# GeekAlexis/FastMOT

Measured on AMD Instinct MI355X. Metric: end-to-end tracker FPS @1080p/50 dets, higher is better.
Workload: dtype f16

## Files before the change

fastmot_amd/csrc/resblock.hip:

```cpp
#include "net.h"
#include <cstdlib>

namespace {

typedef float f32x16 __attribute__((ext_vector_type(16)));

template <int C, int M, int TH, int NW, int CS, int KS>
__global__ __launch_bounds__(NW * 64) void resblock_kernel(
    const f16* __restrict__ x, int x_cs, int x_coff, f16* __restrict__ out, int out_cs, int out_coff,
    const f16* __restrict__ w1, const float* __restrict__ b1, const f16* __restrict__ w2,
    const float* __restrict__ b2, int H, int W, int tiles_x, int act1, int act2) {
    constexpr int TW = 8, HW = TW + 2, NPOS = (TH + 2) * HW, SX = C + 8, S = M + 8, NT = NW * 64;
    constexpr int NMT = M / 32, NPH = (NPOS + 31) / 32, NPAIR = NMT * NPH / NW;
    constexpr int NCT = C / 32 / CS, NPT = TH * TW / 32;
    static_assert(NMT * NPH % NW == 0 && NCT * NPT * KS == NW, "tile / wave split");
    extern __shared__ __attribute__((aligned(16))) f16 lds[];
    f16* xt = lds;
    f16* mid = lds + NPOS * SX;
    const int tid = threadIdx.x, lane = tid & 63, wave = __builtin_amdgcn_readfirstlane(tid >> 6);
    const int frow = lane & 31, fk = (lane >> 5) * 8;
    const int tile = blockIdx.x / CS, cs = blockIdx.x % CS;
    const int ty0 = (tile / tiles_x) * TH, tx0 = (tile % tiles_x) * TW;
    const long n = blockIdx.y;
    const f16* img = x + n * (long)H * W * x_cs + x_coff;

    {
        constexpr int VPP = C / 8, NV = NPOS * VPP, NIT = (NV + NT - 1) / NT;
        f16x8 v[NIT];
#pragma unroll
        for (int i = 0; i < NIT; ++i) {
            const int e = tid + i * NT, pos = e / VPP, c8 = (e % VPP) * 8;
            const int py = ty0 - 1 + pos / HW, px = tx0 - 1 + pos % HW;
            const bool ok = e < NV && py >= 0 && py < H && px >= 0 && px < W;
            const f16x8 ld = *reinterpret_cast<const f16x8*>(
                img + ((long)min(max(py, 0), H - 1) * W + min(max(px, 0), W - 1)) * x_cs + c8);
#pragma unroll
            for (int j = 0; j < 8; ++j) v[i][j] = ok ? ld[j] : (f16)0.f;
        }
#pragma unroll
        for (int i = 0; i < NIT; ++i) {
            const int e = tid + i * NT;
            if (e < NV) *reinterpret_cast<f16x8*>(&xt[(e / VPP) * SX + (e % VPP) * 8]) = v[i];
        }
    }

    {
        constexpr int ST = C / 16, CH1 = ST < 8 ? ST : 8, KC = ST / CH1, NI = NPAIR * KC, PD = NI < 3 ? NI : 3;
        f16x8 fa[PD][CH1];
        float4 bias1[NPAIR][4];
#pragma unroll
        for (int p = 0; p < NPAIR; ++p)
#pragma unroll
            for (int g = 0; g < 4; ++g)
                bias1[p][g] = *reinterpret_cast<const float4*>((const float*)__builtin_assume_aligned(b1, 16) +
                                                               ((wave + p * NW) % NMT) * 32 + g * 8 + (lane >> 5) * 4);
        auto load_a = [&](int item, int slot) {
            const int mt = (wave + (item / KC) * NW) % NMT;
            const f16* wr = w1 + (((long)mt * ST + (item % KC) * CH1) * 64 + lane) * 8;
#pragma unroll
            for (int u = 0; u < CH1; ++u) fa[slot][u] = *reinterpret_cast<const f16x8*>(wr + u * 512);
        };
#pragma unroll
        for (int i = 0; i < PD; ++i) load_a(i, i);
        __syncthreads();
        f32x16 acc;
#pragma unroll
        for (int item = 0; item < NI; ++item) {
            const int p = item / KC, kc = (item % KC) * CH1 * 16;
            const int pos = ((wave + p * NW) / NMT) * 32 + frow;
            const f16* bsrc = xt + min(pos, NPOS - 1) * SX + fk + kc;
            f16x8 fb[CH1];
#pragma unroll
            for (int u = 0; u < CH1; ++u) fb[u] = *reinterpret_cast<const f16x8*>(bsrc + u * 16);
            if (item % KC == 0) {
#pragma unroll
                for (int r = 0; r < 16; ++r) acc[r] = 0.f;
            }
#pragma unroll
            for (int u = 0; u < CH1; ++u) acc = __builtin_amdgcn_mfma_f32_32x32x16_f16(fa[item % PD][u], fb[u], acc, 0, 0, 0);
            if (item + PD < NI) load_a(item + PD, item % PD);
            if (item % KC == KC - 1 && pos < NPOS) {
                const int py = ty0 - 1 + pos / HW, px = tx0 - 1 + pos % HW;
                const bool inside = py >= 0 && py < H && px >= 0 && px < W;
                const int mt = (wave + p * NW) % NMT;
#pragma unroll
                for (int g = 0; g < 4; ++g) {
                    const float4 bv = bias1[p][g];
                    union { f16 h[4]; uint2 u; } pk;
                    float a4[4] = {acc[g * 4 + 0] + bv.x, acc[g * 4 + 1] + bv.y, acc[g * 4 + 2] + bv.z,
                                   acc[g * 4 + 3] + bv.w};
                    apply_act_n<4>(a4, act1);
#pragma unroll
                    for (int e = 0; e < 4; ++e) pk.h[e] = (f16)(inside ? a4[e] : 0.f);
                    *reinterpret_cast<uint2*>(&mid[pos * S + mt * 32 + g * 8 + (lane >> 5) * 4]) = pk.u;
                }
            }
        }
    }

    const int ctl = wave % NCT, pt = (wave / NCT) % NPT, ks = wave / (NCT * NPT);
    const int ct = cs * NCT + ctl;
    const int pix = pt * 32 + frow;
    const int gy = ty0 + pix / TW, gx = tx0 + pix % TW;
    float4 bias2[4];
#pragma unroll
    for (int g = 0; g < 4; ++g)
        bias2[g] = *reinterpret_cast<const float4*>((const float*)__builtin_assume_aligned(b2, 16) + ct * 32 + g * 8 +
                                                    (lane >> 5) * 4);
    f32x16 acc;
    {
        constexpr int SPT = M / 16;
        constexpr int CH = (SPT % 8 == 0 && 9 * SPT % (8 * KS) == 0) ? 8 : (SPT % 4 == 0 && 9 * SPT % (4 * KS) == 0) ? 4 : 2;
        constexpr int NQ = 9 * SPT / CH / KS, PD = NQ < 24 / CH ? NQ : 24 / CH;
        static_assert(SPT % CH == 0 && 9 * SPT % (CH * KS) == 0, "chunking");
        const int q0 = ks * NQ;
        const f16* wr = w2 + (((long)ct * (9 * SPT) + q0 * CH) * 64 + lane) * 8;
        f16x8 fa[PD][CH], fb[2][CH];
        auto load_a = [&](int q, int slot) {
#pragma unroll
            for (int u = 0; u < CH; ++u) fa[slot][u] = *reinterpret_cast<const f16x8*>(wr + (q * CH + u) * 512);
        };
        const int pbase = ((pix / TW) * HW + pix % TW) * S + fk;
        auto load_b = [&](int q, int slot) {
            const int step0 = (q0 + q) * CH, tap = step0 / SPT;
            const f16* src = mid + pbase + ((tap / 3) * HW + tap % 3) * S + (step0 % SPT) * 16;
#pragma unroll
            for (int u = 0; u < CH; ++u) fb[slot][u] = *reinterpret_cast<const f16x8*>(src + u * 16);
        };
#pragma unroll
        for (int i = 0; i < PD; ++i) load_a(i, i);
#pragma unroll
        for (int r = 0; r < 16; ++r) acc[r] = 0.f;
        __syncthreads();
        load_b(0, 0);
#pragma unroll
        for (int q = 0; q < NQ; ++q) {
            if (q + 1 < NQ) load_b(q + 1, (q + 1) & 1);
            __builtin_amdgcn_sched_barrier(0);
#pragma unroll
            for (int u = 0; u < CH; ++u)
                acc = __builtin_amdgcn_mfma_f32_32x32x16_f16(fa[q % PD][u], fb[q & 1][u], acc, 0, 0, 0);
            if (q + PD < NQ) load_a(q + PD, q % PD);
            __builtin_amdgcn_sched_barrier(0);
        }
    }
    if constexpr (KS > 1) {
        float4* red = reinterpret_cast<float4*>(mid);
        __syncthreads();
        if (ks > 0) {
#pragma unroll
            for (int g = 0; g < 4; ++g)
                red[(((ks - 1) * NCT * NPT + ctl + NCT * pt) * 4 + g) * 64 + lane] =
                    make_float4(acc[g * 4], acc[g * 4 + 1], acc[g * 4 + 2], acc[g * 4 + 3]);
        }
        __syncthreads();
        if (ks > 0) return;
#pragma unroll
        for (int k = 1; k < KS; ++k)
#pragma unroll
            for (int g = 0; g < 4; ++g) {
                const float4 v = red[(((k - 1) * NCT * NPT + ctl + NCT * pt) * 4 + g) * 64 + lane];
                acc[g * 4] += v.x; acc[g * 4 + 1] += v.y; acc[g * 4 + 2] += v.z; acc[g * 4 + 3] += v.w;
            }
    }

    if (gy < H && gx < W) {
        const long gp = (n * H + gy) * (long)W + gx;
        const f16* rsrc = xt + ((pix / TW + 1) * HW + pix % TW + 1) * SX;
#pragma unroll
        for (int g = 0; g < 4; ++g) {
            const int co = ct * 32 + g * 8 + (lane >> 5) * 4;
            const f16x4 rv = *reinterpret_cast<const f16x4*>(rsrc + co);
            f16x4 o;
            float a4[4] = {acc[g * 4 + 0] + bias2[g].x, acc[g * 4 + 1] + bias2[g].y, acc[g * 4 + 2] + bias2[g].z,
                           acc[g * 4 + 3] + bias2[g].w};
            apply_act_n<4>(a4, act2);
#pragma unroll
            for (int e = 0; e < 4; ++e) o[e] = (f16)(a4[e] + (float)rv[e]);
            *reinterpret_cast<f16x4*>(out + gp * out_cs + out_coff + co) = o;
        }
    }
}

template <int C, int M, int TH, int NW, int KS>
constexpr size_t resblock_lds() {
    constexpr size_t npos = (TH + 2) * 10, midb = npos * (M + 8) * 2, redb = (size_t)(KS - 1) * (NW / KS) * 64 * 64;
    return npos * (C + 8) * 2 + (midb > redb ? midb : redb);
}

template <int C, int M, int TH, int NW, int CS, int KS>
int resblock_launch(const f16* x, int x_cs, int x_coff, f16* out, int out_cs, int out_coff, const f16* w1,
                    const float* b1, const f16* w2, const float* b2, int N, int H, int W, int act1, int act2,
                    hipStream_t s) {
    const int tiles_x = (W + 7) / 8, tiles_y = (H + TH - 1) / TH;
    constexpr size_t shmem = resblock_lds<C, M, TH, NW, KS>();
    static_assert(shmem <= 64 * 1024, "LDS tile");
    hipLaunchKernelGGL((resblock_kernel<C, M, TH, NW, CS, KS>), dim3(tiles_x * tiles_y * CS, N), dim3(NW * 64), shmem, s, x, x_cs,
                       x_coff, out, out_cs, out_coff, w1, b1, w2, b2, H, W, tiles_x, act1, act2);
    FM_HIP(hipGetLastError());
    return 0;
}

}

bool resblock_supported(int C, int M) {
    return (C == 64 || C == 128 || C == 256) && (M == C || M == C / 2);
}

int launch_resblock(const f16* x, int x_cs, int x_coff, f16* out, int out_cs, int out_coff, const f16* w1,
                    const float* b1, const f16* w2, const float* b2, int N, int H, int W, int C, int M, int act1,
                    int act2, hipStream_t s) {
    FM_CHECK_ARG(resblock_supported(C, M) && x_cs % 8 == 0 && x_coff % 8 == 0 && out_cs % 4 == 0 && out_coff % 4 == 0);
#define RB(C_, M_, TH_, NW_, CS_, KS_)                                                                         \
    if (C == C_ && M == M_)                                                                                    \
        return resblock_launch<C_, M_, TH_, NW_, CS_, KS_>(x, x_cs, x_coff, out, out_cs, out_coff, w1, b1, w2, \
                                                           b2, N, H, W, act1, act2, s)
    static const int variant = getenv("FASTMOT_RB_VARIANT") ? atoi(getenv("FASTMOT_RB_VARIANT")) : 1;
    if (variant == 1) { RB(64, 64, 8, 8, 1, 2); RB(128, 128, 4, 8, 1, 2); }
    if (variant == 2) { RB(128, 128, 8, 8, 1, 1); }
    RB(64, 32, 8, 4, 1, 1);
    RB(64, 64, 8, 4, 1, 1);
    RB(128, 64, 4, 4, 1, 1);
    RB(128, 128, 4, 4, 1, 1);
    RB(256, 128, 4, 8, 4, 4);
    RB(256, 256, 4, 8, 4, 4);
#undef RB
    return FM_ERR_ARG;
}

extern "C" int fm_resblock_supported(int c, int mid) { return resblock_supported(c, mid) ? 1 : 0; }
```

Measured before the change: 1027.

## Add persistent weight-resident resblock kernel with halo prefetch for C=64,M=32

Adds a persistent-style resblock kernel for C=64, M=32. Each block loops over a contiguous range of tiles, keeps both 1x1 and 3x3 weights in registers for the whole range, and prefetches the next tile's halo into registers while the 3x3 MFMA stage runs. The output is staged through LDS so global stores are 16-byte vectors. This is meant to cut repeated weight loads and hide global-load latency, at the cost of more registers and fewer blocks (about 512), which lowers occupancy and parallelism.

```diff
diff --git a/fastmot_amd/csrc/resblock.hip b/fastmot_amd/csrc/resblock.hip
--- a/fastmot_amd/csrc/resblock.hip
+++ b/fastmot_amd/csrc/resblock.hip
@@ -182,6 +182,193 @@
     }
 }
 
+#ifndef FM_RB_SLOTS
+#define FM_RB_SLOTS 512
+#endif
+#ifndef FM_RB_PREFETCH
+#define FM_RB_PREFETCH 1
+#endif
+
+template <int C, int M, int NW, int KS>
+__global__ __launch_bounds__(NW * 64) void resblock_lm_kernel(
+    const f16* __restrict__ x, int x_cs, int x_coff, f16* __restrict__ out, int out_cs, int out_coff,
+    const f16* __restrict__ w1, const float* __restrict__ b1, const f16* __restrict__ w2,
+    const float* __restrict__ b2, int H, int W, int tiles_x, int tiles_img, int tiles_total, int tpw, int act1,
+    int act2) {
+    constexpr int TH = 8, TW = 8, HW = TW + 2, NPOS = (TH + 2) * HW, SX = C + 8, S = M + 8, NT = NW * 64;
+    constexpr int NMT = M / 32, NPH = (NPOS + 31) / 32, NCT = C / 32, NPT = TH * TW / 32;
+    constexpr int ST = C / 16, SPT = M / 16, CH = 2, NQ = 9 * SPT / CH / KS;
+    static_assert(NMT * NPH == NW && NCT * NPT * KS == NW && 9 * SPT % (CH * KS) == 0 && ST == 4, "tile / wave split");
+    static_assert((SPT % 4 != 0 || 9 * SPT % (4 * KS) != 0) && NQ * CH <= 24, "chunking of resblock_kernel");
+    extern __shared__ __attribute__((aligned(16))) f16 lds[];
+    f16* xt = lds;
+    f16* mid = lds + NPOS * SX;
+    const int tid = threadIdx.x, lane = tid & 63, wave = __builtin_amdgcn_readfirstlane(tid >> 6);
+    const int frow = lane & 31, fk = (lane >> 5) * 8;
+    const int t0 = blockIdx.x * tpw, t1 = min(t0 + tpw, tiles_total);
+    if (t0 >= t1) return;
+
+    const int mt = wave % NMT, pos1 = (wave / NMT) * 32 + frow;
+    const int ct = wave % NCT, pt = (wave / NCT) % NPT, ks = wave / (NCT * NPT);
+    const int pix = pt * 32 + frow;
+    f16x8 fa1[ST], fa2[NQ][CH];
+    float4 bias1[4], bias2[4];
+#pragma unroll
+    for (int g = 0; g < 4; ++g) {
+        bias1[g] = *reinterpret_cast<const float4*>((const float*)__builtin_assume_aligned(b1, 16) + mt * 32 + g * 8 + (lane >> 5) * 4);
+        bias2[g] = *reinterpret_cast<const float4*>((const float*)__builtin_assume_aligned(b2, 16) + ct * 32 + g * 8 + (lane >> 5) * 4);
+    }
+#pragma unroll
+    for (int u = 0; u < ST; ++u) fa1[u] = *reinterpret_cast<const f16x8*>(w1 + (((long)mt * ST + u) * 64 + lane) * 8);
+#pragma unroll
+    for (int q = 0; q < NQ; ++q)
+#pragma unroll
+        for (int u = 0; u < CH; ++u)
+            fa2[q][u] = *reinterpret_cast<const f16x8*>(w2 + (((long)ct * (9 * SPT) + (ks * NQ + q) * CH + u) * 64 + lane) * 8);
+
+    constexpr int VPP = C / 8, NV = NPOS * VPP, NIT = (NV + NT - 1) / NT;
+    f16x8 hv[NIT];
+    unsigned hok = 0;
+    auto halo_load = [&](int t) {
+        const int n = t / tiles_img, r = t - n * tiles_img;
+        const int ty0 = (r / tiles_x) * TH, tx0 = (r % tiles_x) * TW;
+        const f16* img = x + (long)n * H * W * x_cs + x_coff;
+        hok = 0;
+#pragma unroll
+        for (int i = 0; i < NIT; ++i) {
+            const int e = tid + i * NT, pos = e / VPP, c8 = (e % VPP) * 8;
+            const int py = ty0 - 1 + pos / HW, px = tx0 - 1 + pos % HW;
+            hok |= (e < NV && py >= 0 && py < H && px >= 0 && px < W ? 1u : 0u) << i;
+            hv[i] = *reinterpret_cast<const f16x8*>(
+                img + ((long)min(max(py, 0), H - 1) * W + min(max(px, 0), W - 1)) * x_cs + c8);
+        }
+    };
+    auto halo_store = [&]() {
+#pragma unroll
+        for (int i = 0; i < NIT; ++i) {
+            const int e = tid + i * NT;
+            f16x8 v = hv[i];
+            if (!((hok >> i) & 1u)) {
+#pragma unroll
+                for (int j = 0; j < 8; ++j) v[j] = (f16)0.f;
+            }
+            if (e < NV) *reinterpret_cast<f16x8*>(&xt[(e / VPP) * SX + (e % VPP) * 8]) = v;
+        }
+    };
+    halo_load(t0);
+
+    for (int t = t0; t < t1; ++t) {
+        const int n = t / tiles_img, r = t - n * tiles_img;
+        const int ty0 = (r / tiles_x) * TH, tx0 = (r % tiles_x) * TW;
+        if (!FM_RB_PREFETCH && t > t0) halo_load(t);
+        halo_store();
+        __syncthreads();
+
+        {
+            const f16* bsrc = xt + min(pos1, NPOS - 1) * SX + fk;
+            f16x8 fb[ST];
+#pragma unroll
+            for (int u = 0; u < ST; ++u) fb[u] = *reinterpret_cast<const f16x8*>(bsrc + u * 16);
+            f32x16 acc;
+#pragma unroll
+            for (int r16 = 0; r16 < 16; ++r16) acc[r16] = 0.f;
+#pragma unroll
+            for (int u = 0; u < ST; ++u) acc = __builtin_amdgcn_mfma_f32_32x32x16_f16(fa1[u], fb[u], acc, 0, 0, 0);
+            if (pos1 < NPOS) {
+                const int py = ty0 - 1 + pos1 / HW, px = tx0 - 1 + pos1 % HW;
+                const bool inside = py >= 0 && py < H && px >= 0 && px < W;
+#pragma unroll
+                for (int g = 0; g < 4; ++g) {
+                    const float4 bv = bias1[g];
+                    union { f16 h[4]; uint2 u; } pk;
+                    float a4[4] = {acc[g * 4 + 0] + bv.x, acc[g * 4 + 1] + bv.y, acc[g * 4 + 2] + bv.z,
+                                   acc[g * 4 + 3] + bv.w};
+                    apply_act_n<4>(a4, act1);
+#pragma unroll
+                    for (int e = 0; e < 4; ++e) pk.h[e] = (f16)(inside ? a4[e] : 0.f);
+                    *reinterpret_cast<uint2*>(&mid[pos1 * S + mt * 32 + g * 8 + (lane >> 5) * 4]) = pk.u;
+                }
+            }
+        }
+        __syncthreads();
+        if (FM_RB_PREFETCH && t + 1 < t1) halo_load(t + 1);
+
+        f32x16 acc;
+        {
+            f16x8 fb[2][CH];
+            const int pbase = ((pix / TW) * HW + pix % TW) * S + fk;
+            auto load_b = [&](int q, int slot) {
+                const int step0 = (ks * NQ + q) * CH, tap = step0 / SPT;
+                const f16* src = mid + pbase + ((tap / 3) * HW + tap % 3) * S + (step0 % SPT) * 16;
+#pragma unroll
+                for (int u = 0; u < CH; ++u) fb[slot][u] = *reinterpret_cast<const f16x8*>(src + u * 16);
+            };
+#pragma unroll
+            for (int r16 = 0; r16 < 16; ++r16) acc[r16] = 0.f;
+            load_b(0, 0);
+#pragma unroll
+            for (int q = 0; q < NQ; ++q) {
+                if (q + 1 < NQ) load_b(q + 1, (q + 1) & 1);
+                __builtin_amdgcn_sched_barrier(0);
+#pragma unroll
+                for (int u = 0; u < CH; ++u)
+                    acc = __builtin_amdgcn_mfma_f32_32x32x16_f16(fa2[q][u], fb[q & 1][u], acc, 0, 0, 0);
+                __builtin_amdgcn_sched_barrier(0);
+            }
+        }
+        if constexpr (KS > 1) {
+            float4* red = reinterpret_cast<float4*>(mid);
+            __syncthreads();
+            if (ks > 0) {
+#pragma unroll
+                for (int g = 0; g < 4; ++g)
+                    red[(((ks - 1) * NCT * NPT + ct + NCT * pt) * 4 + g) * 64 + lane] =
+                        make_float4(acc[g * 4], acc[g * 4 + 1], acc[g * 4 + 2], acc[g * 4 + 3]);
+            }
+            __syncthreads();
+            if (ks == 0) {
+#pragma unroll
+                for (int k = 1; k < KS; ++k)
+#pragma unroll
+                    for (int g = 0; g < 4; ++g) {
+                        const float4 v = red[(((k - 1) * NCT * NPT + ct + NCT * pt) * 4 + g) * 64 + lane];
+                        acc[g * 4] += v.x; acc[g * 4 + 1] += v.y; acc[g * 4 + 2] += v.z; acc[g * 4 + 3] += v.w;
+                    }
+            }
+        }
+
+        if (ks == 0) {
+            f16* rsrc = xt + ((pix / TW + 1) * HW + pix % TW + 1) * SX;
+#pragma unroll
+            for (int g = 0; g < 4; ++g) {
+                const int co = ct * 32 + g * 8 + (lane >> 5) * 4;
+                const f16x4 rv = *reinterpret_cast<const f16x4*>(rsrc + co);
+                f16x4 o;
+                float a4[4] = {acc[g * 4 + 0] + bias2[g].x, acc[g * 4 + 1] + bias2[g].y, acc[g * 4 + 2] + bias2[g].z,
+                               acc[g * 4 + 3] + bias2[g].w};
+                apply_act_n<4>(a4, act2);
+#pragma unroll
+                for (int e = 0; e < 4; ++e) o[e] = (f16)(a4[e] + (float)rv[e]);
+                *reinterpret_cast<f16x4*>(rsrc + co) = o;
+            }
+        }
+        __syncthreads();
+        {
+            constexpr int NO = TH * TW * VPP;
+            static_assert(NO % NT == 0, "output pieces per thread");
+#pragma unroll
+            for (int i = 0; i < NO / NT; ++i) {
+                const int e = tid + i * NT, p = e / VPP, c8 = (e % VPP) * 8;
+                const int gy = ty0 + p / TW, gx = tx0 + p % TW;
+                if (gy < H && gx < W)
+                    *reinterpret_cast<f16x8*>(out + (((long)n * H + gy) * W + gx) * out_cs + out_coff + c8) =
+                        *reinterpret_cast<const f16x8*>(&xt[((p / TW + 1) * HW + p % TW + 1) * SX + c8]);
+            }
+        }
+        if (t + 1 < t1) __syncthreads();
+    }
+}
+
 template <int C, int M, int TH, int NW, int KS>
 constexpr size_t resblock_lds() {
     constexpr size_t npos = (TH + 2) * 10, midb = npos * (M + 8) * 2, redb = (size_t)(KS - 1) * (NW / KS) * 64 * 64;
@@ -201,6 +388,23 @@
     return 0;
 }
 
+template <int C, int M, int NW, int KS>
+int resblock_lm_launch(const f16* x, int x_cs, int x_coff, f16* out, int out_cs, int out_coff, const f16* w1,
+                       const float* b1, const f16* w2, const float* b2, int N, int H, int W, int act1, int act2,
+                       hipStream_t s) {
+    const int tiles_x = (W + 7) / 8, tiles_img = tiles_x * ((H + 7) / 8);
+    const long total = (long)tiles_img * N;
+    FM_CHECK_ARG(total < (1L << 30));
+    const int tpw = (int)((total + FM_RB_SLOTS - 1) / FM_RB_SLOTS);
+    constexpr size_t shmem = resblock_lds<C, M, 8, NW, KS>();
+    static_assert(shmem <= 64 * 1024, "LDS tile");
+    hipLaunchKernelGGL((resblock_lm_kernel<C, M, NW, KS>), dim3((unsigned)((total + tpw - 1) / tpw)), dim3(NW * 64), shmem, s, x,
+                       x_cs, x_coff, out, out_cs, out_coff, w1, b1, w2, b2, H, W, tiles_x, tiles_img, (int)total, tpw, act1,
+                       act2);
+    FM_HIP(hipGetLastError());
+    return 0;
+}
+
 }
 
 bool resblock_supported(int C, int M) {
@@ -216,6 +420,16 @@
         return resblock_launch<C_, M_, TH_, NW_, CS_, KS_>(x, x_cs, x_coff, out, out_cs, out_coff, w1, b1, w2, \
                                                            b2, N, H, W, act1, act2, s)
     static const int variant = getenv("FASTMOT_RB_VARIANT") ? atoi(getenv("FASTMOT_RB_VARIANT")) : 1;
+#ifndef FM_RB_NO_LM
+    if (C == 64 && out_cs % 8 == 0 && out_coff % 8 == 0 && variant == 1) {
+#define RBL(M_, NW_, KS_)                                                                                                  \
+    if (M == M_)                                                                                                           \
+        return resblock_lm_launch<64, M_, NW_, KS_>(x, x_cs, x_coff, out, out_cs, out_coff, w1, b1, w2, b2, N, H, W, act1, \
+                                                    act2, s)
+        RBL(32, 4, 1);
+#undef RBL
+    }
+#endif
     if (variant == 1) { RB(64, 64, 8, 8, 1, 2); RB(128, 128, 4, 8, 1, 2); }
     if (variant == 2) { RB(128, 128, 8, 8, 1, 1); }
     RB(64, 32, 8, 4, 1, 1);
```

New measurement: 993.5. 3.3% lower.
